# rapidsai/cugraph-gnn

Hardware: AMD Instinct MI355X
Metric: sampled-edges/sec (sample+renumber+feature-gather+SAGEConv fwd), ogbn-products-like fan-out [25, 10] (higher is better)
Workload: dtype int64 ids (int32 timed as a variant) + f32 features (SAGE lin_l/lin_r product: bf16x3-split MFMA, f32 accumulate)

## Files before the change

cugraph-gnn_amd/csrc/wg_rng.hpp:

```cpp
#pragma once
#include <hip/hip_runtime.h>

#include <cstdint>

namespace wgamd {

struct PcgJump {
  uint64_t a;
  uint64_t s;
};

struct PcgJumpTables {
  PcgJump t[4][256];
  constexpr PcgJumpTables() : t{}
  {
    uint64_t base_a = 6364136223846793005ULL, base_s = 1;
    for (int k = 0; k < 4; k++) {
      t[k][0].a = 1;
      t[k][0].s = 0;
      for (int c = 1; c < 256; c++) {
        t[k][c].a = t[k][c - 1].a * base_a;
        t[k][c].s = t[k][c - 1].s * base_a + base_s;
      }
      for (int d = 0; d < 8; d++) {
        uint64_t na = base_a * base_a, ns = base_s * base_a + base_s;
        base_a = na;
        base_s = ns;
      }
    }
  }
};

__device__ __constant__ const PcgJumpTables g_pcg_jump{};

struct Pcg32 {
  uint64_t state;
  uint64_t inc;

  static constexpr uint64_t kMult = 6364136223846793005ULL;

  __host__ __device__ __forceinline__ uint32_t next_u32()
  {
    uint64_t old = state;
    state        = old * kMult + inc;
    uint32_t x   = (uint32_t)(((old >> 18u) ^ old) >> 27u);
    uint32_t rot = (uint32_t)(old >> 59u);
    return (x >> rot) | (x << ((0u - rot) & 31u));
  }

  __host__ __device__ __forceinline__ void skipahead(uint64_t delta)
  {
    uint64_t acc_mult = 1u, acc_plus = 0u, cur_mult = kMult, cur_plus = inc;
    while (delta) {
      if (delta & 1u) {
        acc_mult *= cur_mult;
        acc_plus = acc_plus * cur_mult + cur_plus;
      }
      cur_plus = (cur_mult + 1u) * cur_plus;
      cur_mult *= cur_mult;
      delta >>= 1u;
    }
    state = acc_mult * state + acc_plus;
  }

  __host__ __device__ __forceinline__ Pcg32(uint64_t seed, uint64_t subsequence)
  {
    state = 0u;
    inc   = (subsequence << 1u) | 1u;
    (void)next_u32();
    state += seed;
    (void)next_u32();
    skipahead(subsequence);
  }

  __device__ __forceinline__ void jump_table(uint32_t n)
  {
    PcgJump j = g_pcg_jump.t[0][n & 255u];
#pragma unroll
    for (int k = 1; k < 4; k++) {
      const uint32_t c = (n >> (8 * k)) & 255u;
      if (c) {
        const PcgJump m = g_pcg_jump.t[k][c];
        j.s             = j.s * m.a + m.s;
        j.a             = j.a * m.a;
      }
    }
    state = j.a * state + inc * j.s;
  }

  struct table_tag {};
  __device__ __forceinline__ Pcg32(uint64_t seed, uint32_t subsequence, table_tag, uint32_t extra_draws = 0)
  {
    inc   = ((uint64_t)subsequence << 1u) | 1u;
    state = (inc + seed) * kMult + inc;
    jump_table(subsequence + extra_draws);
  }

  __host__ __device__ __forceinline__ int32_t next_i31() { return (int32_t)(next_u32() & 0x7fffffffu); }
  __host__ __device__ __forceinline__ uint64_t next_u64()
  {
    uint64_t lo = next_u32();
    uint64_t hi = next_u32();
    return lo | (hi << 32u);
  }
  __host__ __device__ __forceinline__ int64_t next_i63() { return (int64_t)(next_u64() & 0x7fffffffffffffffULL); }
  __host__ __device__ __forceinline__ float next_f32() { return (float)(next_u32() >> 8u) / 16777216.0f; }
};

}
```

cugraph-gnn_amd/csrc/wg_sample.hip:

```cpp
#include <algorithm>
#include <cmath>

#include "wg_common.hpp"
#include "wg_rng.hpp"

namespace wgamd {
namespace {

template <typename T>
struct dtype_of;
template <>
struct dtype_of<int32_t> {
  static constexpr wholememory_dtype_t value = WHOLEMEMORY_DT_INT;
};
template <>
struct dtype_of<int64_t> {
  static constexpr wholememory_dtype_t value = WHOLEMEMORY_DT_INT64;
};

__host__ __device__ constexpr int ref_block_threads(int M)
{
  int f = (M - 1) / 32;
  return f < 3 ? 32 : f < 6 ? 64 : f < 12 ? 128 : 256;
}
// ... 14 lines not shown
  const int64_t sid = seed_index * B + lane;
  if (sid < (1ll << 31)) return Pcg32(random_seed, (uint32_t)sid, Pcg32::table_tag{});
  return Pcg32(random_seed, stream_id(seed_index, B, lane));
}

constexpr int kWaveRowCapDecl = 1024;
constexpr int kHugeRow = 16384;

template <typename SeedT>
__global__ void __launch_bounds__(256) sample_count_kernel(const int64_t* __restrict__ row_ptr,
                                                           const SeedT* __restrict__ seeds,
                                                           dev_count n_,
                                                           int M,
                                                           int* __restrict__ cnt,
                                                           int* __restrict__ big_deg ,
                                                           int* __restrict__ lists = nullptr ,
                                                           int list_cap            = 0,
                                                           int scratch_threshold   = 0,
                                                           int64_t* __restrict__ row_start = nullptr,
                                                           int* __restrict__ row_deg       = nullptr)
{
  const int n_live = n_.get();
  if (lists == nullptr) {
    const int end = min(n_.host, (n_live / kScanTile + 1) * kScanTile);
    for (int i = blockIdx.x * blockDim.x + threadIdx.x; i < end; i += gridDim.x * blockDim.x) {
      int deg = 0;
      if (i < n_live) {
        const int64_t nid   = (int64_t)seeds[i];
        const int64_t first = row_ptr[nid];
        deg                 = (int)(row_ptr[nid + 1] - first);
        if (row_start) {
          row_start[i] = first;
          row_deg[i]   = deg;
        }
        deg = (M > 0 && deg > M) ? M : deg;
      }
      cnt[i] = deg;
      if (big_deg) big_deg[i] = 0;
    }
    return;
  }
  int i = blockIdx.x * blockDim.x + threadIdx.x;
  int cls          = -1;
  int deg          = 0;
  if (i < n_.host) {
    if (i >= n_live) {
      if (i < (n_live / kScanTile + 1) * kScanTile) {
        cnt[i] = 0;
        if (big_deg) big_deg[i] = 0;
      }
    } else {
      int64_t nid         = (int64_t)seeds[i];
      const int64_t first = row_ptr[nid];
      deg                 = (int)(row_ptr[nid + 1] - first);
      cnt[i]              = (M > 0 && deg > M) ? M : deg;
      if (row_start) {
        row_start[i] = first;
        row_deg[i]   = deg;
      }
      if (big_deg) big_deg[i] = 0;
      if (lists != nullptr && M > 0 && deg > M) {
        cls = deg <= 16 ? 0 : deg <= 32 ? 1 : deg <= 64 ? 2 : deg <= 128 ? 3 : deg <= 256 ? 4 : deg <= 512 ? 5
              : deg <= kWaveRowCapDecl ? 6 : deg <= kHugeRow ? 7 : 8;
        if (cls >= 7 && deg > scratch_threshold) atomicMax(lists + 10, deg);
      }
    }
  }
  if (lists == nullptr) return;
  __shared__ int blk_cnt[kWeightedLists], blk_base[kWeightedLists];
  if (threadIdx.x < kWeightedLists) blk_cnt[threadIdx.x] = 0;
  __syncthreads();
  const int lane = threadIdx.x & 63;
  int my_rank    = 0;
#pragma unroll
  for (int c = 0; c < kWeightedLists; c++) {
    const uint64_t m = __ballot(cls == c);
    if (m == 0ull) continue;
    const int leader = __ffsll((long long)m) - 1;
    int base         = 0;
    if (lane == leader) base = atomicAdd(&blk_cnt[c], __popcll(m));
    base = __shfl(base, leader, 64);
    if (cls == c) my_rank = base + __popcll(m & ((1ull << lane) - 1ull));
  }
  __syncthreads();
  if (threadIdx.x < kWeightedLists && blk_cnt[threadIdx.x] > 0) blk_base[threadIdx.x] = atomicAdd(lists + threadIdx.x, blk_cnt[threadIdx.x]);
  __syncthreads();
  if (cls >= 0) lists[kWeightedListHead + (int64_t)cls * list_cap + blk_base[cls] + my_rank] = i;
}

template <typename ColT>
__device__ __forceinline__ ColT col_at(const ColT* __restrict__ col, int64_t at)
{
  return col ? col[at] : (ColT)0;
}

constexpr int kWalkGrid = 256 * 16;

template <typename ColT>
__device__ __forceinline__ void emit(ColT* dst, int* src_lid, int64_t* edge_gid, int64_t out, ColT v,
                                     int seed_index, int64_t gid)
{
  if (dst) dst[out] = v;
  if (src_lid) src_lid[out] = seed_index;
  if (edge_gid) edge_gid[out] = gid;
}

struct loc_rec {
  int64_t start;
  int i;
  int deg;
  int base;
  int i_local;
  int batch;
  int pad;
};
static_assert(sizeof(loc_rec) == 32, "one 32-byte sector per record");
constexpr int kLocBuckets = 4096;
constexpr int kLocBlocks  = 128;
constexpr int kLocThreads = 1024;

template <typename SeedT>
__global__ void __launch_bounds__(kLocThreads)
locality_hist_kernel(const SeedT* __restrict__ seeds, dev_count n_, int shift, int* __restrict__ hist )
{
  __shared__ int h[kLocBuckets];
  const int n = n_.get(), per = (n + kLocBlocks - 1) / kLocBlocks;
  const int lo = min(n, (int)blockIdx.x * per), hi = min(n, lo + per);
  for (int k = threadIdx.x; k < kLocBuckets; k += kLocThreads) h[k] = 0;
  __syncthreads();
  for (int i = lo + threadIdx.x; i < hi; i += kLocThreads)
    atomicAdd(&h[min((int)((uint64_t)seeds[i] >> shift), kLocBuckets - 1)], 1);
  __syncthreads();
  for (int k = threadIdx.x; k < kLocBuckets; k += kLocThreads) hist[(int64_t)blockIdx.x * kLocBuckets + k] = h[k];
}

template <typename SeedT>
__global__ void __launch_bounds__(kLocThreads)
locality_scatter_kernel(const SeedT* __restrict__ seeds, dev_count n_, int shift, const int* __restrict__ hist,
                        const int64_t* __restrict__ row_start, const int* __restrict__ row_deg, const int* __restrict__ offsets,
                        rng_plan rng, loc_rec* __restrict__ recs)
{
  __shared__ int cursor[kLocBuckets];
  __shared__ int wave_tot[kLocThreads / 64];
  static_assert(kLocBuckets == 4 * kLocThreads, "thread t owns buckets 4 t .. 4 t + 3");
  const int n = n_.get(), per = (n + kLocBlocks - 1) / kLocBlocks;
  const int lo = min(n, (int)blockIdx.x * per), hi = min(n, lo + per);
  int tot[4] = {0, 0, 0, 0}, before[4] = {0, 0, 0, 0};
  const int4* h4 = reinterpret_cast<const int4*>(hist);
  for (int b = 0; b < kLocBlocks; b++) {
    const int4 v = h4[(int64_t)b * (kLocBuckets / 4) + threadIdx.x];
    tot[0] += v.x; tot[1] += v.y; tot[2] += v.z; tot[3] += v.w;
    if (b < (int)blockIdx.x) { before[0] += v.x; before[1] += v.y; before[2] += v.z; before[3] += v.w; }
  }
  const int sum = tot[0] + tot[1] + tot[2] + tot[3];
  int inc = sum;
  const int lane = threadIdx.x & 63, wave = threadIdx.x >> 6;
#pragma unroll
  for (int d = 1; d < 64; d <<= 1) {
    const int up = __shfl_up(inc, d, 64);
    if (lane >= d) inc += up;
  }
  if (lane == 63) wave_tot[wave] = inc;
  __syncthreads();
  int run = inc - sum;
  for (int w = 0; w < wave; w++) run += wave_tot[w];
#pragma unroll
  for (int k = 0; k < 4; k++) {
    cursor[4 * threadIdx.x + k] = run + before[k];
    run += tot[k];
  }
  __syncthreads();
  for (int i = lo + threadIdx.x; i < hi; i += kLocThreads) {
    const int j = atomicAdd(&cursor[min((int)((uint64_t)seeds[i] >> shift), kLocBuckets - 1)], 1);
    loc_rec r;
    r.start = row_start[i];
    r.i     = i;
    r.deg   = row_deg[i];
    r.base  = offsets[i];
    r.i_local = i;
    r.batch   = 0;
    if (rng.target_batch) {
      r.batch   = rng.target_batch[i];
      r.i_local = i - rng.target_seg[r.batch];
    }
    r.pad   = 0;
    recs[j] = r;
  }
}

template <typename SeedT, typename ColT, int LANES>
__global__ void __launch_bounds__(256) sample_uniform_halfwave_kernel(const int64_t* __restrict__ row_ptr,
                                                                      const ColT* __restrict__ col,
                                                                      const SeedT* __restrict__ seeds,
                                                                      dev_count n_,
                                                                      int M,
                                                                      rng_plan rng,
                                                                      const int* __restrict__ offsets,
                                                                      ColT* __restrict__ dst,
                                                                      int* __restrict__ src_lid,
                                                                      int64_t* __restrict__ edge_gid,
                                                                      const int64_t* __restrict__ row_start,
                                                                      const int* __restrict__ row_deg,
                                                                      const loc_rec* __restrict__ recs = nullptr)
{
  const int n    = n_.get();
  const int lane = threadIdx.x & 63;
  const int hl   = lane & (LANES - 1);
  const int hb   = lane & ~(LANES - 1);
  int i          = (int)(((int64_t)blockIdx.x * blockDim.x + threadIdx.x) / LANES);
  loc_rec rec{};
  if (recs) {
    constexpr int kGroups = 256 / LANES;
    const int per_x = ((n + 7) / 8 + kGroups - 1) / kGroups * kGroups;
    const int k     = (int)(blockIdx.x >> 3) * kGroups + (int)threadIdx.x / LANES;
    const int j     = (int)(blockIdx.x & 7) * per_x + k;
    i               = n;
    if (k < per_x && j < n) {
      rec = recs[j];
      i   = rec.i;
    }
  }
  int32_t r_draw = 0;
  if (i < n && hl < M) {
    uint64_t random_seed;
    int i_local;
    if (recs) {
      i_local     = rec.i_local;
      random_seed = rng.seeds_dev ? rng.seeds_dev[rec.batch] : rng.seed;
    } else
      rng.resolve(i, random_seed, i_local);
    if (i_local < (1 << 26)) {
      Pcg32 g(random_seed, (uint32_t)(i_local * 32 + hl), Pcg32::table_tag{});
      r_draw = g.next_i31();
    } else {
      Pcg32 g(random_seed, stream_id(i_local, 32, hl));
      r_draw = g.next_i31();
    }
  }
  int64_t start = 0;
  int N = 0, base = 0;
  if (i < n && recs) {
    start = rec.start;
    N     = rec.deg;
    base  = rec.base;
  } else if (i < n) {
    if (row_start) {
      start = row_start[i];
      N     = row_deg[i];
    } else {
      int64_t nid = (int64_t)seeds[i];
      start       = row_ptr[nid];
      N           = (int)(row_ptr[nid + 1] - start);
    }
    base = offsets[i];
  }
  const bool pick = N > M;
  if (__ballot(pick) == 0ull) {
    if (hl < N) emit<ColT>(dst, src_lid, edge_gid, (int64_t)base + hl, col_at<ColT>(col, start + hl), i, start + hl);
    return;
  }
  int r = 0;
  if (pick && hl < M) r = r_draw % (N - hl);
  const int tail = N - hl - 1;
  int p1 = -1, p2 = -1;
  for (int s = 0; s + 1 < M; s++) {
    const int rs    = __shfl(r, hb | s, 64);
    const bool prev = s < hl;
    p1 = (prev && rs == r) ? s : p1;
    p2 = (prev && rs == tail) ? s : p2;
  }
  int root = p2 >= 0 ? p2 : hl;
#pragma unroll
  for (int round = 0; round < (LANES == 32 ? 5 : 4); round++) root = __shfl(root, hb | root, 64);
  const int val = N - root - 1;
  const int vp1 = __shfl(val, hb | (p1 & (LANES - 1)), 64);
  const int a   = p1 >= 0 ? vp1 : r;
  if (pick) {
    if (hl < M) emit<ColT>(dst, src_lid, edge_gid, (int64_t)base + hl, col_at<ColT>(col, start + a), i, start + a);
  } else if (hl < N) {
    emit<ColT>(dst, src_lid, edge_gid, (int64_t)base + hl, col_at<ColT>(col, start + hl), i, start + hl);
  }
}

template <typename SeedT, typename ColT, int GW, int K, bool EXACT>
__global__ void __launch_bounds__(256)
sample_uniform_multi_kernel(const ColT* __restrict__ col, dev_count n_, int M_rt, rng_plan rng, const int* __restrict__ offsets,
                            ColT* __restrict__ dst, int* __restrict__ src_lid, int64_t* __restrict__ edge_gid,
                            const int64_t* __restrict__ row_start, const int* __restrict__ row_deg,
                            const loc_rec* __restrict__ recs)
{
  constexpr int kGPW    = 64 / GW;
  constexpr int kGroups = 4 * kGPW;
  constexpr int kRounds = GW <= 2 ? 1 : GW <= 4 ? 2 : GW <= 8 ? 3 : GW <= 16 ? 4 : 5;
  const int M    = EXACT ? GW : M_rt;
  const int n    = n_.get();
  const int lane = threadIdx.x & 63;
  const int grp  = lane / GW;
  const int hl   = lane - grp * GW;
  const int hb   = grp * GW;
  const bool live_group = grp < kGPW;
  const int wg_group    = (int)(threadIdx.x >> 6) * kGPW + grp;
  const int per_x = ((n + 7) / 8 + kGroups * K - 1) / (kGroups * K) * (kGroups * K);
  const int64_t n_chunks = recs ? (int64_t)(per_x / (kGroups * K)) * 8 : ((int64_t)n + kGroups * K - 1) / (kGroups * K);
  for (int64_t chunk = blockIdx.x; chunk < n_chunks; chunk += gridDim.x) {
  int i[K], N[K], base[K], i_local[K], batch[K];
  int64_t start[K];
  if (recs) {
    const int k0    = ((int)(chunk >> 3) * kGroups + wg_group) * K;
#pragma unroll
    for (int k = 0; k < K; k++) {
      const int j = (int)(chunk & 7) * per_x + k0 + k;
      i[k] = n, N[k] = 0, base[k] = 0, start[k] = 0, i_local[k] = 0, batch[k] = 0;
      if (live_group && k0 + k < per_x && j < n) {
        const loc_rec r = recs[j];
        i[k] = r.i, N[k] = r.deg, base[k] = r.base, start[k] = r.start, i_local[k] = r.i_local, batch[k] = r.batch;
      }
    }
  } else {
    const int64_t g = chunk * kGroups + wg_group;
#pragma unroll
    for (int k = 0; k < K; k++) {
      i[k] = live_group ? (int)min(g * K + k, (int64_t)n) : n;
      N[k] = 0, base[k] = 0, start[k] = 0, i_local[k] = i[k], batch[k] = 0;
      if (i[k] < n) {
        start[k] = row_start[i[k]];
        N[k]     = row_deg[i[k]];
        base[k]  = offsets[i[k]];
        if (rng.target_batch) batch[k] = rng.target_batch[i[k]];
      }
    }
    if (rng.target_batch) {
#pragma unroll
      for (int k = 0; k < K; k++)
        if (i[k] < n) i_local[k] = i[k] - rng.target_seg[batch[k]];
    }
  }
  int32_t r_draw[K];
#pragma unroll
  for (int k = 0; k < K; k++) {
    r_draw[k] = 0;
    if (i[k] < n && hl < M) {
      const uint64_t random_seed = rng.seeds_dev ? rng.seeds_dev[rng.target_batch ? batch[k] : 0] : rng.seed;
      if (i_local[k] < (1 << 26)) {
        Pcg32 g(random_seed, (uint32_t)(i_local[k] * 32 + hl), Pcg32::table_tag{});
        r_draw[k] = g.next_i31();
      } else {
        Pcg32 g(random_seed, stream_id(i_local[k], 32, hl));
        r_draw[k] = g.next_i31();
      }
    }
  }
  int a[K];
#pragma unroll
  for (int k = 0; k < K; k++) {
    const bool pick = N[k] > M;
    a[k]            = hl;
    if (__ballot(pick) != 0ull) {
      int r = 0;
      if (pick && hl < M) r = r_draw[k] % (N[k] - hl);
      const int tail = N[k] - hl - 1;
      int p1 = -1, p2 = -1;
      auto step = [&](int s) {
        const int rs    = __shfl(r, hb + s, 64);
        const bool prev = s < hl;
        p1 = (prev && rs == r) ? s : p1;
        p2 = (prev && rs == tail) ? s : p2;
      };
      if constexpr (EXACT) {
#pragma unroll
        for (int s = 0; s + 1 < GW; s++) step(s);
      } else {
        for (int s = 0; s + 1 < M; s++) step(s);
      }
      int root = p2 >= 0 ? p2 : hl;
#pragma unroll
      for (int round = 0; round < kRounds; round++) root = __shfl(root, hb + root, 64);
      const int val = N[k] - root - 1;
      const int vp1 = __shfl(val, hb + max(p1, 0), 64);
      if (pick) a[k] = p1 >= 0 ? vp1 : r;
    }
  }
  ColT v[K];
  bool on[K];
#pragma unroll
  for (int k = 0; k < K; k++) {
    on[k] = live_group && hl < (N[k] > M ? M : N[k]);
    v[k]  = on[k] ? col_at<ColT>(col, start[k] + a[k]) : (ColT)0;
  }
#pragma unroll
  for (int k = 0; k < K; k++)
    if (on[k]) emit<ColT>(dst, src_lid, edge_gid, (int64_t)base[k] + hl, v[k], i[k], start[k] + a[k]);
  }
}

constexpr int kHashSlots = 4096;

__device__ __forceinline__ int lds_hash_find(const int* keys, int pos)
{
  uint32_t h = ((uint32_t)pos * 2654435761u) & (kHashSlots - 1);
  while (true) {
    int k = keys[h];
    if (k == pos || k == -1) return (int)h;
    h = (h + 1) & (kHashSlots - 1);
  }
}

template <typename SeedT, typename ColT>
__global__ void __launch_bounds__(256) sample_uniform_block_kernel(const int64_t* __restrict__ row_ptr,
                                                                   const ColT* __restrict__ col,
                                                                   const SeedT* __restrict__ seeds,
                                                                   dev_count n_,
                                                                   int M,
                                                                   int B,
                                                                   int items,
                                                                   rng_plan rng,
                                                                   const int* __restrict__ offsets,
                                                                   ColT* __restrict__ dst,
                                                                   int* __restrict__ src_lid,
                                                                   int64_t* __restrict__ edge_gid)
{
  __shared__ int r[1024];
  __shared__ int a[1024];
  __shared__ int hkeys[kHashSlots];
  __shared__ int hvals[kHashSlots];
  const int i = blockIdx.x;
  if (i >= n_.get()) return;
  const int64_t nid   = (int64_t)seeds[i];
  const int64_t start = row_ptr[nid];
  const int N         = (int)(row_ptr[nid + 1] - start);
  if (N <= 0) return;
  const int base = offsets[i];
  if (N <= M) {
    for (int j = threadIdx.x; j < N; j += blockDim.x)
      emit<ColT>(dst, src_lid, edge_gid, (int64_t)base + j, col_at<ColT>(col, start + j), i, start + j);
    return;
  }
  for (int h = threadIdx.x; h < kHashSlots; h += blockDim.x) hkeys[h] = -1;
  if ((int)threadIdx.x < B) {
    uint64_t random_seed;
    int i_local;
    rng.resolve(i, random_seed, i_local);
    Pcg32 g(random_seed, stream_id(i_local, B, threadIdx.x));
    for (int k = 0; k < items; k++) {
      int id = k * B + threadIdx.x;
      int v  = g.next_i31();
      if (id < M) r[id] = v % (N - id);
    }
  }
  __syncthreads();
  if (threadIdx.x == 0) {
    for (int t = 0; t < M; t++) {
      const int rt = r[t], tail = N - t - 1;
      int s1     = lds_hash_find(hkeys, rt);
      int q_rt   = hkeys[s1] == rt ? hvals[s1] : rt;
      int s2     = lds_hash_find(hkeys, tail);
      int q_tail = hkeys[s2] == tail ? hvals[s2] : tail;
      a[t]       = q_rt;
      hkeys[s1]  = rt;
      hvals[s1]  = q_tail;
    }
  }
  __syncthreads();
  for (int t = threadIdx.x; t < M; t += blockDim.x)
    emit<ColT>(dst, src_lid, edge_gid, (int64_t)base + t, col_at<ColT>(col, start + a[t]), i, start + a[t]);
}

template <typename SeedT, typename ColT>
__global__ void __launch_bounds__(64) sample_uniform_reservoir_kernel(const int64_t* __restrict__ row_ptr,
                                                                      const ColT* __restrict__ col,
                                                                      const SeedT* __restrict__ seeds,
                                                                      dev_count n_,
                                                                      int M,
                                                                      rng_plan rng,
                                                                      const int* __restrict__ offsets,
                                                                      ColT* __restrict__ dst,
                                                                      int* __restrict__ src_lid,
                                                                      int64_t* __restrict__ edge_gid)
{
  const int i = blockIdx.x;
  if (i >= n_.get()) return;
  const int64_t nid   = (int64_t)seeds[i];
  const int64_t start = row_ptr[nid];
  const int N         = (int)(row_ptr[nid + 1] - start);
  if (N <= 0) return;
  const int64_t base = offsets[i];
  if (N <= M) {
    for (int j = threadIdx.x; j < N; j += blockDim.x)
      emit<ColT>(dst, src_lid, edge_gid, base + j, col_at<ColT>(col, start + j), i, start + j);
    return;
  }
  for (int s = threadIdx.x; s < M; s += blockDim.x) dst[base + s] = (ColT)s;
  __syncthreads();
  if (threadIdx.x < 32) {
    uint64_t random_seed;
    int i_local;
    rng.resolve(i, random_seed, i_local);
    Pcg32 g(random_seed, stream_id(i_local, 32, threadIdx.x));
    for (int idx = M + threadIdx.x; idx < N; idx += 32) {
      int rn = g.next_i31() % (idx + 1);
      if (rn < M) {
        if constexpr (sizeof(ColT) == 8)
          atomicMax(reinterpret_cast<long long*>(dst + base + rn), (long long)idx);
        else
          atomicMax(reinterpret_cast<int*>(dst + base + rn), idx);
      }
    }
  }
  __syncthreads();
  for (int s = threadIdx.x; s < M; s += blockDim.x) {
    int sel = (int)__hip_atomic_load(dst + base + s, __ATOMIC_RELAXED, __HIP_MEMORY_SCOPE_AGENT);
    emit<ColT>(dst, src_lid, edge_gid, base + s, col_at<ColT>(col, start + sel), i, start + sel);
  }
}

__device__ __forceinline__ float ares_key(float w, Pcg32& g, bool* redrawn = nullptr)
{
  float u = g.next_f32();
  u       = (float)(-(0.5 + 0.5 * (double)u));
  uint64_t x;
  int zero_draws = -1;
  do {
    x = g.next_u64();
    zero_draws++;
  } while (!x);
  if (redrawn != nullptr && zero_draws > 0) *redrawn = true;
  int one_bit = __clzll((long long)x) + zero_draws * 64;
  u *= exp2f((float)(-one_bit));
#ifdef WG_TUNE_CHEAP_KEY
  return u * 1.442695f * __builtin_amdgcn_rcpf(w);
#endif
  return (log1pf(u) / logf(2.0f)) * (1.0f / w);
}

constexpr int kWaveRowCap = 1024;
static_assert(kWaveRowCap == kWaveRowCapDecl, "keep the two in step");

__device__ __forceinline__ uint32_t key_bits(float k)
{
  uint32_t b = __float_as_uint(k);
  return (b & 0x80000000u) ? ~b : (b | 0x80000000u);
}

constexpr int kLdsKeys = kWeightedLdsKeys;

template <typename SeedT, typename ColT, typename WeightT, int B, int T>
__global__ void __launch_bounds__(T) sample_weighted_kernel(const int64_t* __restrict__ row_ptr,
                                                            const ColT* __restrict__ col,
                                                            const WeightT* __restrict__ weight,
                                                            const SeedT* __restrict__ seeds,
                                                            dev_count n_,
                                                            int M,
                                                            rng_plan rng,
                                                            const int* __restrict__ offsets,
                                                            uint32_t* __restrict__ slab,
                                                            int64_t slab_len,
                                                            ColT* __restrict__ dst,
                                                            int* __restrict__ src_lid,
                                                            int64_t* __restrict__ edge_gid,
                                                            int* __restrict__ lists ,
                                                            int list_cap,
                                                            int redo = 0 )
{
  static_assert(T % B == 0 && T % 64 == 0, "threads must be a multiple of the stream layout and of the wave");
  __shared__ uint32_t lds_keys[kLdsKeys];
  __shared__ int hist[256];
  __shared__ int sh_digit, sh_need, sh_redo;
  __shared__ int wave_cnt[2][T / 64];
  __shared__ int sh_li;
  const int n_live  = n_.get();
  const int n_huge  = lists && !redo ? lists[8] : 0;
  const int count   = lists ? (redo ? lists[kWeightedRedoCount] : n_huge + lists[7]) : n_live;
  uint32_t* gkeys   = slab + (int64_t)blockIdx.x * slab_len;
  int li            = blockIdx.x;
  while (true) {
  __syncthreads();
  if (lists) {
    if (threadIdx.x == 0) sh_li = atomicAdd(lists + (redo ? kWeightedRedoHead : 9), 1);
    __syncthreads();
    li = sh_li;
  }
  if (li >= count) break;
  const int i = lists ? (redo ? lists[kWeightedListHead + (int64_t)kWeightedRedoList * list_cap + li]
                         : li < n_huge ? lists[kWeightedListHead + 8 * (int64_t)list_cap + li]
                                       : lists[kWeightedListHead + 7 * (int64_t)list_cap + (li - n_huge)])
                      : li;
  if (!lists) li += gridDim.x;
  if (i >= n_live) continue;
  uint64_t random_seed;
  int i_rng;
  rng.resolve(i, random_seed, i_rng);
  const int64_t nid   = (int64_t)seeds[i];
  const int64_t start = row_ptr[nid];
  const int N         = (int)(row_ptr[nid + 1] - start);
  if (N <= 0) continue;
  const int64_t base = offsets[i];
  if (M <= 0 || N <= M) {
    for (int j = threadIdx.x; j < N; j += T)
      emit<ColT>(dst, src_lid, edge_gid, base + j, col_at<ColT>(col, start + j), i, start + j);
    continue;
  }
  const bool in_lds = N <= kLdsKeys;
  auto put = [&](int id, uint32_t k) { if (in_lds) lds_keys[id] = k; else gkeys[id] = k; };
  auto get = [&](int id) -> uint32_t {
    return in_lds ? lds_keys[id] : __hip_atomic_load(gkeys + id, __ATOMIC_RELAXED, __HIP_MEMORY_SCOPE_AGENT);
  };
  if (threadIdx.x == 0) sh_redo = 0;
  __syncthreads();
  {
    constexpr int hop = T / B;
    const int lane = threadIdx.x % B, part = threadIdx.x / B;
    const int L     = lane < N ? (N - lane + B - 1) / B : 0;
    const int share = (L + hop - 1) / hop;
    const int m0 = part * share, m1 = min(L, m0 + share);
    bool redrawn = false;
    if (m0 < m1) {
      const int64_t sid = (int64_t)i_rng * B + lane;
      Pcg32 g = (sid < (1ll << 31)) ? Pcg32(random_seed, (uint32_t)sid, Pcg32::table_tag{}, 3u * (uint32_t)m0)
                                    : Pcg32(random_seed, stream_id(i_rng, B, lane));
      if (sid >= (1ll << 31)) g.skipahead(3u * (uint64_t)m0);
      for (int m = m0; m < m1; m++) {
        const int id = lane + m * B;
        put(id, key_bits(ares_key((float)weight[start + id], g, &redrawn)));
      }
    }
    if (redrawn) sh_redo = 1;
  }
  __syncthreads();
  if (T > B && sh_redo) {
    if (threadIdx.x < B) {
      Pcg32 g = stream_generator(random_seed, i_rng, B, threadIdx.x);
      for (int id = threadIdx.x; id < N; id += B) put(id, key_bits(ares_key((float)weight[start + id], g)));
    }
    __syncthreads();
  }
  uint32_t prefix = 0, prefix_mask = 0;
  int need = M;
  for (int shift = 24; shift >= 0; shift -= 8) {
    for (int h = threadIdx.x; h < 256; h += T) hist[h] = 0;
    __syncthreads();
    for (int id = threadIdx.x; id < N; id += T) {
      uint32_t k = get(id);
      if ((k & prefix_mask) == prefix) atomicAdd(&hist[(k >> shift) & 255], 1);
    }
    __syncthreads();
    if (threadIdx.x < 64) {
      const int l  = threadIdx.x;
      const int h0 = hist[4 * l], h1 = hist[4 * l + 1], h2 = hist[4 * l + 2], h3 = hist[4 * l + 3];
      const int own = h0 + h1 + h2 + h3;
      int inc = own;
      for (int off = 1; off < 64; off <<= 1) {
        int v = __shfl_down(inc, off);
        if (l + off < 64) inc += v;
      }
// ... 1246 lines not shown
```

Baseline: 5.308 billion.

## Compute per-row PCG jump once per group and share it via LDS

Splits the PCG table-jump into a row-dependent part (seed times the jump for i<<5), computed once per sampled row by one lane and shared through a per-wave LDS slot array, and a lane-dependent part taken from small table constants. Each lane then produces its first draw with a closed-form affine combination instead of a full 4-level constant-table jump. This is meant to remove redundant 64-bit multiplies and constant-memory lookups repeated by all GW lanes of a group. In exchange it adds shuffles, LDS traffic, wave barriers and an asm trick to keep the lane index in a vector register.

```diff
diff --git a/cugraph-gnn_amd/csrc/wg_rng.hpp b/cugraph-gnn_amd/csrc/wg_rng.hpp
--- a/cugraph-gnn_amd/csrc/wg_rng.hpp
+++ b/cugraph-gnn_amd/csrc/wg_rng.hpp
@@ -33,6 +33,51 @@
 
 __device__ __constant__ const PcgJumpTables g_pcg_jump{};
 
+__host__ __device__ __forceinline__ uint32_t pcg_xsh_rr(uint64_t old)
+{
+  const uint32_t x   = (uint32_t)(((old >> 18u) ^ old) >> 27u);
+  const uint32_t rot = (uint32_t)(old >> 59u);
+  return (x >> rot) | (x << ((0u - rot) & 31u));
+}
+
+__device__ __forceinline__ PcgJump pcg_jump(uint32_t n)
+{
+  PcgJump j = g_pcg_jump.t[0][n & 255u];
+#pragma unroll
+  for (int k = 1; k < 4; k++) {
+    const uint32_t c = (n >> (8 * k)) & 255u;
+    if (c) {
+      const PcgJump m = g_pcg_jump.t[k][c];
+      j.s             = j.s * m.a + m.s;
+      j.a             = j.a * m.a;
+    }
+  }
+  return j;
+}
+
+struct PcgLane32 {
+  uint64_t a1;
+  uint64_t a2;
+  uint64_t s2;
+};
+
+__device__ __forceinline__ PcgLane32 pcg_lane32(int h)
+{
+  return {g_pcg_jump.t[0][h + 1].a, g_pcg_jump.t[0][h + 2].a, g_pcg_jump.t[0][h + 2].s};
+}
+
+__device__ __forceinline__ PcgJump pcg_seed32(uint64_t seed, uint32_t i)
+{
+  const PcgJump j = pcg_jump(i << 5);
+  return {j.a * seed, j.s};
+}
+
+__device__ __forceinline__ int32_t pcg_first_i31_lane32(const PcgJump& sj, uint32_t i, int h, const PcgLane32& c)
+{
+  const uint32_t inc = (i << 6) | (uint32_t)(2 * h + 1);
+  return (int32_t)(pcg_xsh_rr(sj.a * c.a1 + (uint64_t)inc * (sj.s * c.a2 + c.s2)) & 0x7fffffffu);
+}
+
 struct Pcg32 {
   uint64_t state;
   uint64_t inc;
@@ -41,11 +86,9 @@
 
   __host__ __device__ __forceinline__ uint32_t next_u32()
   {
-    uint64_t old = state;
-    state        = old * kMult + inc;
-    uint32_t x   = (uint32_t)(((old >> 18u) ^ old) >> 27u);
-    uint32_t rot = (uint32_t)(old >> 59u);
-    return (x >> rot) | (x << ((0u - rot) & 31u));
+    const uint64_t old = state;
+    state              = old * kMult + inc;
+    return pcg_xsh_rr(old);
   }
 
   __host__ __device__ __forceinline__ void skipahead(uint64_t delta)
@@ -75,17 +118,8 @@
 
   __device__ __forceinline__ void jump_table(uint32_t n)
   {
-    PcgJump j = g_pcg_jump.t[0][n & 255u];
-#pragma unroll
-    for (int k = 1; k < 4; k++) {
-      const uint32_t c = (n >> (8 * k)) & 255u;
-      if (c) {
-        const PcgJump m = g_pcg_jump.t[k][c];
-        j.s             = j.s * m.a + m.s;
-        j.a             = j.a * m.a;
-      }
-    }
-    state = j.a * state + inc * j.s;
+    const PcgJump j = pcg_jump(n);
+    state           = j.a * state + inc * j.s;
   }
 
   struct table_tag {};
diff --git a/cugraph-gnn_amd/csrc/wg_sample.hip b/cugraph-gnn_amd/csrc/wg_sample.hip
--- a/cugraph-gnn_amd/csrc/wg_sample.hip
+++ b/cugraph-gnn_amd/csrc/wg_sample.hip
@@ -340,6 +340,8 @@
   const int wg_group    = (int)(threadIdx.x >> 6) * kGPW + grp;
   const int per_x = ((n + 7) / 8 + kGroups * K - 1) / (kGroups * K) * (kGroups * K);
   const int64_t n_chunks = recs ? (int64_t)(per_x / (kGroups * K)) * 8 : ((int64_t)n + kGroups * K - 1) / (kGroups * K);
+  static_assert(kGPW * K <= 64, "one seed slot per lane");
+  __shared__ PcgJump seed_half[256];
   for (int64_t chunk = blockIdx.x; chunk < n_chunks; chunk += gridDim.x) {
   int i[K], N[K], base[K], i_local[K], batch[K];
   int64_t start[K];
@@ -374,19 +376,39 @@
     }
   }
   int32_t r_draw[K];
-#pragma unroll
-  for (int k = 0; k < K; k++) {
-    r_draw[k] = 0;
-    if (i[k] < n && hl < M) {
-      const uint64_t random_seed = rng.seeds_dev ? rng.seeds_dev[rng.target_batch ? batch[k] : 0] : rng.seed;
-      if (i_local[k] < (1 << 26)) {
-        Pcg32 g(random_seed, (uint32_t)(i_local[k] * 32 + hl), Pcg32::table_tag{});
-        r_draw[k] = g.next_i31();
-      } else {
-        Pcg32 g(random_seed, stream_id(i_local[k], 32, hl));
-        r_draw[k] = g.next_i31();
-      }
-    }
+  {
+    const int qg = lane % kGPW, qk = lane / kGPW;
+    int q_il = 0, q_b = 0;
+#pragma unroll
+    for (int k = 0; k < K; k++) {
+      const int il = __shfl(i_local[k], qg * GW, 64);
+      const int b  = __shfl(batch[k], qg * GW, 64);
+      q_il         = qk == k ? il : q_il;
+      q_b          = qk == k ? b : q_b;
+    }
+    PcgJump q_sj{0, 0};
+    if (qk < K && (uint32_t)q_il < (1u << 26))
+      q_sj = pcg_seed32(rng.seeds_dev ? rng.seeds_dev[rng.target_batch ? q_b : 0] : rng.seed, (uint32_t)q_il);
+    PcgJump* row = seed_half + (threadIdx.x & ~63);
+    row[lane]    = q_sj;
+    __builtin_amdgcn_wave_barrier();
+    int h_opaque = hl;
+    asm volatile("" : "+v"(h_opaque));
+    const PcgLane32 lane_c = pcg_lane32(h_opaque);
+#pragma unroll
+    for (int k = 0; k < K; k++) {
+      r_draw[k] = 0;
+      if (i[k] < n && hl < M) {
+        if ((uint32_t)i_local[k] < (1u << 26)) {
+          r_draw[k] = pcg_first_i31_lane32(row[k * kGPW + grp], (uint32_t)i_local[k], hl, lane_c);
+        } else {
+          const uint64_t random_seed = rng.seeds_dev ? rng.seeds_dev[rng.target_batch ? batch[k] : 0] : rng.seed;
+          Pcg32 g(random_seed, stream_id(i_local[k], 32, hl));
+          r_draw[k] = g.next_i31();
+        }
+      }
+    }
+    __builtin_amdgcn_wave_barrier();
   }
   int a[K];
 #pragma unroll
```

Result: no change. 5.301 billion (median of 6 runs) (-0.1%).
